# trnKhanh/medical-image-analysis

Measured on AMD Instinct MI355X. Metric: training images/sec (whole node), UNet 512x512 1ch bs=32/GPU, higher is better.
Workload: dtype bf16; 1 GPU; UNet-2D channels [64, 128, 256, 512, 1024] 512x512 1ch, batch 32/GPU, instance norm, dropout 0.1, Dice+CE, Adam(wd 5e-4), clip 10 (cfg3); global_batch=32, parallelism=dp1

## Files before the change

medical-image-analysis_amd/csrc/common.h:

```cpp
#pragma once
#include <hip/hip_runtime.h>
#include <stdint.h>
#include <stdio.h>
#include <string.h>

#define MIA_F32 0
#define MIA_BF16 1

#define MIA_OK 0
#define MIA_EARG (-1)
#define MIA_EUNSUPPORTED (-2)

extern "C" const char* mia_last_error(void);
void mia_set_error(const char* fmt, ...);

#define MIA_CHECK_ARG(cond, ...)            \
  do {                                      \
    if (!(cond)) {                          \
      mia_set_error(__VA_ARGS__);           \
      return MIA_EARG;                      \
    }                                       \
  } while (0)

#define MIA_LAUNCH_CHECK()                                                  \
// ... 134 lines not shown

__device__ __forceinline__ float wave_sum(float v) {
#pragma unroll
  for (int o = 32; o > 0; o >>= 1) v += __shfl_xor(v, o, 64);
  return v;
}

__device__ __forceinline__ double wave_sum_d(double v) {
#pragma unroll
  for (int o = 32; o > 0; o >>= 1) v += __shfl_xor(v, o, 64);
  return v;
}

__device__ __forceinline__ int wave_sum_i(int v) {
#pragma unroll
  for (int o = 32; o > 0; o >>= 1) v += __shfl_xor(v, o, 64);
  return v;
}

__device__ __forceinline__ float block_sum(float v, float* red ) {
  v = wave_sum(v);
  const int w = threadIdx.x >> 6, l = threadIdx.x & 63, nw = (blockDim.x + 63) >> 6;
  __syncthreads();
  if (l == 0) red[w] = v;
  __syncthreads();
  float r = 0.f;
  if (threadIdx.x < 64) {
    r = (l < nw) ? red[l] : 0.f;
    r = wave_sum(r);
  }
  return r;
}

static inline int ceil_div(int a, int b) { return (a + b - 1) / b; }
static inline int64_t ceil_div64(int64_t a, int64_t b) { return (a + b - 1) / b; }
```

medical-image-analysis_amd/csrc/head.hip:

```cpp
#include "common.h"

#define MAXK 8

template <typename T>
__global__ void head_fwd_kernel(const T* __restrict__ x, const float* __restrict__ w, const float* __restrict__ b,
                                float* __restrict__ out, int64_t npix, int c0, int k1, int64_t osp, int64_t osk,
                                int64_t osn, int64_t hw, bool vec) {
  extern __shared__ float wsh[];
  for (int i = threadIdx.x; i < k1 * c0; i += blockDim.x) wsh[i] = w[i];
  __syncthreads();
  constexpr int EPU = Elem<T>::EPU;
  const int sub = threadIdx.x & 7;
  for (int64_t p = ((int64_t)blockIdx.x * blockDim.x + threadIdx.x) >> 3; p < npix; p += ((int64_t)gridDim.x * blockDim.x) >> 3) {
    float acc[MAXK];
#pragma unroll
    for (int k = 0; k < MAXK; ++k) acc[k] = 0.f;
    const T* row = x + p * c0;
    if (vec) {
      for (int u = sub; u < c0 / EPU; u += 8) {
        alignas(16) T v[EPU];
        *reinterpret_cast<u32x4*>(v) = *reinterpret_cast<const u32x4*>(row + u * EPU);
#pragma unroll
        for (int e = 0; e < EPU; ++e) {
          const float xv = Elem<T>::ld(v + e);
#pragma unroll
          for (int k = 0; k < MAXK; ++k)
            if (k < k1) acc[k] += xv * wsh[k * c0 + u * EPU + e];
        }
      }
    } else {
      for (int ch = sub; ch < c0; ch += 8) {
        const float xv = Elem<T>::ld(row + ch);
#pragma unroll
// ... 164 lines not shown
  return upp;
}
#define HEAD_DISPATCH(KERNEL, T, grid, ...)                                                                           \
  do {                                                                                                                \
    if (upp == 4) {                                                                                                   \
      if (k1 == 2) hipLaunchKernelGGL((KERNEL<T, 2, 4>), grid, dim3(256), 0, st, __VA_ARGS__);                        \
      else if (k1 == 3) hipLaunchKernelGGL((KERNEL<T, 3, 4>), grid, dim3(256), 0, st, __VA_ARGS__);                   \
      else hipLaunchKernelGGL((KERNEL<T, 4, 4>), grid, dim3(256), 0, st, __VA_ARGS__);                                \
    } else if (upp == 8) {                                                                                            \
      if (k1 == 2) hipLaunchKernelGGL((KERNEL<T, 2, 8>), grid, dim3(256), 0, st, __VA_ARGS__);                        \
      else if (k1 == 3) hipLaunchKernelGGL((KERNEL<T, 3, 8>), grid, dim3(256), 0, st, __VA_ARGS__);                   \
      else hipLaunchKernelGGL((KERNEL<T, 4, 8>), grid, dim3(256), 0, st, __VA_ARGS__);                                \
    } else {                                                                                                          \
      if (k1 == 2) hipLaunchKernelGGL((KERNEL<T, 2, 16>), grid, dim3(256), 0, st, __VA_ARGS__);                       \
      else if (k1 == 3) hipLaunchKernelGGL((KERNEL<T, 3, 16>), grid, dim3(256), 0, st, __VA_ARGS__);                  \
      else hipLaunchKernelGGL((KERNEL<T, 4, 16>), grid, dim3(256), 0, st, __VA_ARGS__);                               \
    }                                                                                                                 \
  } while (0)

#define HEAD_DISPATCH_N(KERNEL, T, grid, ...)                                                                         \
  do {                                                                                                                \
    if (upp == 12) {                                                                                                  \
      if (k1 == 2) hipLaunchKernelGGL((KERNEL<T, 2, 16, 12>), grid, dim3(256), 0, st, __VA_ARGS__);                   \
      else if (k1 == 3) hipLaunchKernelGGL((KERNEL<T, 3, 16, 12>), grid, dim3(256), 0, st, __VA_ARGS__);              \
      else hipLaunchKernelGGL((KERNEL<T, 4, 16, 12>), grid, dim3(256), 0, st, __VA_ARGS__);                           \
    } else HEAD_DISPATCH(KERNEL, T, grid, __VA_ARGS__);                                                               \
  } while (0)


template <typename T, int K1, int UPP, int CU = UPP>
__global__ __launch_bounds__(256) void head_norm_fwd_kernel(const T* __restrict__ y, const float* __restrict__ scale,
                                                            const float* __restrict__ shift, float slope,
                                                            const float* __restrict__ w, const float* __restrict__ b,
                                                            float* __restrict__ out, int hw, int slabs, int64_t osn,
                                                            int64_t osp, int64_t osk) {
  constexpr int EPU = Elem<T>::EPU, C0 = CU * EPU, LANES = 256 / UPP;
  const int u = threadIdx.x % UPP, pl = threadIdx.x / UPP;
  const bool act = CU == UPP || u < CU;
  const u32x4 zero4 = {0u, 0u, 0u, 0u};
  const int n = blockIdx.x / slabs, s = blockIdx.x % slabs;
  const int per = (hw + slabs - 1) / slabs, r0 = s * per, r1 = r0 + per < hw ? r0 + per : hw;
  float wr[K1][EPU], sc[EPU], sf[EPU];
#pragma unroll
  for (int e = 0; e < EPU; ++e) {
    sc[e] = act ? scale[(size_t)n * C0 + u * EPU + e] : 0.f;
    sf[e] = act ? shift[(size_t)n * C0 + u * EPU + e] : 0.f;
#pragma unroll
    for (int k = 0; k < K1; ++k) wr[k][e] = act ? w[k * C0 + u * EPU + e] : 0.f;
  }
  float bu = 0.f;
#pragma unroll
  for (int k = 0; k < K1; ++k) bu = (u == k) ? b[k] : bu;
  const T* yb = y + (size_t)n * hw * C0 + u * EPU;
  float* ob = out + (int64_t)n * osn + u * osk;
  auto body = [&](const u32x4& raw, int p) {
    alignas(16) T v[EPU];
    *reinterpret_cast<u32x4*>(v) = raw;
    float acc[K1];
#pragma unroll
    for (int k = 0; k < K1; ++k) acc[k] = 0.f;
#pragma unroll
    for (int e = 0; e < EPU; ++e) {
      float xv = sc[e] * Elem<T>::ld(v + e) + sf[e];
      xv = xv > 0.f ? xv : xv * slope;
#pragma unroll
      for (int k = 0; k < K1; ++k) acc[k] += xv * wr[k][e];
    }
    float mine = 0.f;
#pragma unroll
    for (int k = 0; k < K1; ++k) { const float t = group_sum<UPP>(acc[k]); mine = (u == k) ? t : mine; }
    if (u < K1) ob[(int64_t)p * osp] = mine + bu;
  };
  constexpr int GP = 64 / UPP;
  __shared__ float tbuf[4][K1][64];
// ... 326 lines not shown
    if (dtype == MIA_BF16) {
      if (dx) hipLaunchKernelGGL(head_bwd_input_vec_kernel<bf16_t>, dim3(vblocks), dim3(256), k1 * c0 * 4, st, dlogits, w, static_cast<bf16_t*>(dx), npix, c0, k1, gsp, gsk, gsn, hw);
      if (wg) { hipLaunchKernelGGL(head_bwd_weight_vec_kernel<bf16_t>, dim3(wblocks), dim3(256), (256 / (c0 / epu)) * (c0 + 1) * 4, st, dlogits, static_cast<const bf16_t*>(x), workspace, npix, c0, k1, gsp, gsk, gsn, hw); }
    } else {
      if (dx) hipLaunchKernelGGL(head_bwd_input_vec_kernel<float>, dim3(vblocks), dim3(256), k1 * c0 * 4, st, dlogits, w, static_cast<float*>(dx), npix, c0, k1, gsp, gsk, gsn, hw);
      if (wg) { hipLaunchKernelGGL(head_bwd_weight_vec_kernel<float>, dim3(wblocks), dim3(256), (256 / (c0 / epu)) * (c0 + 1) * 4, st, dlogits, static_cast<const float*>(x), workspace, npix, c0, k1, gsp, gsk, gsn, hw); }
    }
  } else if (dtype == MIA_BF16) {
    if (dx) hipLaunchKernelGGL(head_bwd_input_kernel<bf16_t>, dim3(blocks), dim3(256), k1 * c0 * 4, st, dlogits, w, static_cast<bf16_t*>(dx), npix, c0, k1, gsp, gsk, gsn, hw);
    if (wg) { hipLaunchKernelGGL(head_bwd_weight_kernel<bf16_t>, dim3(wblocks), dim3(256), 512 * 4, st, dlogits, static_cast<const bf16_t*>(x), workspace, npix, c0, k1, gsp, gsk, gsn, hw); }
  } else if (dtype == MIA_F32) {
    if (dx) hipLaunchKernelGGL(head_bwd_input_kernel<float>, dim3(blocks), dim3(256), k1 * c0 * 4, st, dlogits, w, static_cast<float*>(dx), npix, c0, k1, gsp, gsk, gsn, hw);
    if (wg) { hipLaunchKernelGGL(head_bwd_weight_kernel<float>, dim3(wblocks), dim3(256), 512 * 4, st, dlogits, static_cast<const float*>(x), workspace, npix, c0, k1, gsp, gsk, gsn, hw); }
  } else { mia_set_error("mia_head_bwd: bad dtype"); return MIA_EARG; }
  if (wg) { hipLaunchKernelGGL(head_bwd_final_kernel, dim3(ceil_div(k1 * (c0 + 1), 16)), dim3(256), 0, st, workspace, wblocks, k1, c0, dw, db, accumulate); }
  MIA_LAUNCH_CHECK();
  return MIA_OK;
}

extern "C" int mia_head_norm_eligible(int dtype, int n, int64_t hw, int c0, int k1) {
  const int epu = dtype == MIA_BF16 ? 8 : 4;
  if ((dtype != MIA_BF16 && dtype != MIA_F32) || c0 % epu != 0) return 0;
  const int upp = c0 / epu;
  if ((upp != 4 && upp != 8 && upp != 12 && upp != 16) || k1 < 2 || k1 > 4) return 0;
  if (hw >= ((int64_t)1 << 31) || n > HEAD_BWD_BLOCKS) return 0;
  return upp;
}
static int head_norm_slabs(int n, int64_t hw) {
  int64_t sl = HEAD_BWD_BLOCKS / n;
  const int64_t maxsl = hw / 512 > 0 ? hw / 512 : 1;
  if (sl > maxsl) sl = maxsl;
  return (int)(sl < 1 ? 1 : sl);
}

extern "C" int mia_head_norm_fwd(const void* y, int dtype, const float* scale, const float* shift, float slope, const float* w,
                                 const float* b, float* logits, int n, int64_t hw, int c0, int k1, int64_t osn, int64_t osk,
                                 int64_t osp, void* stream) {
  MIA_CHECK_ARG(y && scale && shift && w && b && logits && n > 0 && hw > 0, "mia_head_norm_fwd: bad arguments");
  const int upp = mia_head_norm_eligible(dtype, n, hw, c0, k1);
  MIA_CHECK_ARG(upp > 0 && (reinterpret_cast<uintptr_t>(y) & 15) == 0, "mia_head_norm_fwd: shape not eligible (c0=%d k1=%d)", c0, k1);
  hipStream_t st = static_cast<hipStream_t>(stream);
  const int slabs = head_norm_slabs(n, hw);
  if (dtype == MIA_BF16) HEAD_DISPATCH_N(head_norm_fwd_kernel, bf16_t, dim3(n * slabs), static_cast<const bf16_t*>(y), scale, shift, slope, w, b, logits, (int)hw, slabs, osn, osp, osk);
  else HEAD_DISPATCH_N(head_norm_fwd_kernel, float, dim3(n * slabs), static_cast<const float*>(y), scale, shift, slope, w, b, logits, (int)hw, slabs, osn, osp, osk);
  MIA_LAUNCH_CHECK();
  return MIA_OK;
}

extern "C" int mia_head_norm_wgrad(const float* dlogits, const void* y, int dtype, const float* scale, const float* shift,
                                   float slope, float* dw, float* db, float* workspace, int n, int64_t hw, int c0, int k1,
                                   int64_t gsn, int64_t gsk, int64_t gsp, int accumulate, void* stream) {
  MIA_CHECK_ARG(dlogits && y && scale && shift && dw && db && workspace && n > 0 && hw > 0, "mia_head_norm_wgrad: bad arguments");
  const int upp = mia_head_norm_eligible(dtype, n, hw, c0, k1);
  MIA_CHECK_ARG(upp > 0 && (reinterpret_cast<uintptr_t>(y) & 15) == 0, "mia_head_norm_wgrad: shape not eligible (c0=%d k1=%d)", c0, k1);
  hipStream_t st = static_cast<hipStream_t>(stream);
  const int slabs = head_norm_slabs(n, hw);
  if (dtype == MIA_BF16) HEAD_DISPATCH_N(head_norm_wgrad_kernel, bf16_t, dim3(n * slabs), dlogits, static_cast<const bf16_t*>(y), scale, shift, slope, workspace, (int)hw, slabs, gsn, gsp, gsk);
  else HEAD_DISPATCH_N(head_norm_wgrad_kernel, float, dim3(n * slabs), dlogits, static_cast<const float*>(y), scale, shift, slope, workspace, (int)hw, slabs, gsn, gsp, gsk);
  hipLaunchKernelGGL(head_bwd_final_kernel, dim3(ceil_div(k1 * (c0 + 1), 16)), dim3(256), 0, st, workspace, n * slabs, k1, c0, dw, db, accumulate);
  MIA_LAUNCH_CHECK();
  return MIA_OK;
}
```

medical-image-analysis_amd/csrc/norm.hip:

```cpp
#include "common.h"
#include "options.h"
#include <stdlib.h>

#define NORM_INSTANCE 0
#define NORM_BATCH 1

template <bool INST>
__global__ __launch_bounds__(1024) void norm_fwd_sum_kernel(const float* __restrict__ part, int tiles, int c, float* __restrict__ xa, float* __restrict__ xb,
                                    int64_t hw, const float* __restrict__ drop, const float* __restrict__ gamma,
                                    const float* __restrict__ beta, float eps, float* __restrict__ scale, float* __restrict__ shift,
                                    float* __restrict__ ysum) {
  __shared__ double sh1[16][17], sh2[16][17];
  const int cl = threadIdx.x & 15, tl = threadIdx.x >> 4;
  const int n = blockIdx.x, ch = blockIdx.y * 16 + cl;
  double s1 = 0.0, s2 = 0.0;
  if (ch < c) {
    typedef float f2_t __attribute__((ext_vector_type(2)));
    const f2_t* p = reinterpret_cast<const f2_t*>(part) + (size_t)n * tiles * c + ch;
    int t = tl;
    for (; t + 192 < tiles; t += 256) {
      const f2_t v0 = p[(size_t)t * c], v1 = p[(size_t)(t + 64) * c], v2 = p[(size_t)(t + 128) * c], v3 = p[(size_t)(t + 192) * c];
      s1 += (double)v0.x + (double)v1.x + (double)v2.x + (double)v3.x;
      s2 += (double)v0.y + (double)v1.y + (double)v2.y + (double)v3.y;
    }
// ... 871 lines not shown
    float gv[K1];
#pragma unroll
    for (int k = 0; k < K1; ++k) gv[k] = gb[(int64_t)r * gsp + k * gsk];
    body(*reinterpret_cast<const u32x4*>(yb + (size_t)r * c), gv);
  }
#pragma unroll
  for (int e = 0; e < EPU; ++e) { sh[0][pl][u * EPU + e] = s1[e]; sh[1][pl][u * EPU + e] = s2[e]; }
  __syncthreads();
  if (threadIdx.x < 2 * CG) {
    const int k = threadIdx.x / CG, chl = threadIdx.x % CG;
    float t = 0.f;
#pragma unroll 8
    for (int j = 0; j < LANES; ++j) t += sh[k][j][chl];
    part[(((size_t)n * slabs + s) * c + blockIdx.y * CG + chl) * 2 + k] = t;
  }
  if constexpr (HWG) {
#pragma unroll
    for (int k = 0; k < K1; ++k) {
      __syncthreads();
#pragma unroll
      for (int e = 0; e < EPU; ++e) sh[0][pl][u * EPU + e] = wacc[k][e];
      if (u == 0) sh[0][pl][CG] = bacc[k];
      __syncthreads();
      if (threadIdx.x <= CG) {
        float t = 0.f;
#pragma unroll 8
        for (int j = 0; j < LANES; ++j) t += sh[0][j][threadIdx.x];
        wpart[((size_t)blockIdx.x * K1 + k) * (CG + 1) + threadIdx.x] = t;
      }
    }
  }
}

__global__ void head_w_final_kernel(const float* __restrict__ part, int nblk, int k1, int c0, float* __restrict__ dw, float* __restrict__ db,
                                    int accumulate) {
  __shared__ float sh[16][17];
  const int cl = threadIdx.x & 15, tl = threadIdx.x >> 4;
  const int i = blockIdx.x * 16 + cl, tot = k1 * (c0 + 1);
  float sm = 0.f;
  if (i < tot)
    for (int b = tl; b < nblk; b += 16) sm += part[(size_t)b * tot + i];
  sh[tl][cl] = sm;
  __syncthreads();
  if (tl == 0 && i < tot) {
    float t = 0.f;
    for (int j = 0; j < 16; ++j) t += sh[j][cl];
    const int kk = i / (c0 + 1), ch = i % (c0 + 1);
    if (ch < c0) dw[kk * c0 + ch] = accumulate ? dw[kk * c0 + ch] + t : t;
    else db[kk] = accumulate ? db[kk] + t : t;
  }
}



template <typename T, int K1>
__global__ __launch_bounds__(256) void norm_act_bwd_stream_head_kernel(const float* __restrict__ dl, const float* __restrict__ w,
                                                                       const T* __restrict__ y, T* __restrict__ dy,
                                                                       const float* __restrict__ scale, const float* __restrict__ shift,
                                                                       const float* __restrict__ xa, const float* __restrict__ xb,
                                                                       const float* __restrict__ c1, const float* __restrict__ c2,
                                                                       int hw, int c, int slabs, int upb, float slope, int64_t gsn,
                                                                       int64_t gsp, int64_t gsk, unsigned* __restrict__ amax) {
  constexpr int EPU = Elem<T>::EPU;
  const int n = blockIdx.x / slabs, s = blockIdx.x % slabs;
  const int lanes = 256 / upb;
  const int u = blockIdx.y * upb + threadIdx.x % upb, pl = threadIdx.x / upb;
  const bool live = u * EPU < c;
  if (!live && (sizeof(T) != 4 || amax == nullptr)) return;
  const int per = (hw + slabs - 1) / slabs, r0 = s * per, r1 = live ? (r0 + per < hw ? r0 + per : hw) : r0;
  float sc[EPU], sf[EPU], ka[EPU], kb[EPU], wr[K1][EPU];
  unsigned am = 0;
#pragma unroll
  for (int e = 0; e < EPU; ++e) {
    const size_t o = live ? (size_t)n * c + u * EPU + e : 0;
    sc[e] = scale[o]; sf[e] = shift[o];
    ka[e] = -sc[e] * c2[o] * xa[o];
    kb[e] = -sc[e] * (c1[o] + c2[o] * xb[o]);
#pragma unroll
    for (int k = 0; k < K1; ++k) wr[k][e] = live ? w[k * c + u * EPU + e] : 0.f;
// ... 21 lines not shown
  for (; r + 3 * lanes < r1; r += 4 * lanes) {
    u32x4 raw[4];
    float gv[4][K1];
#pragma unroll
    for (int j = 0; j < 4; ++j) raw[j] = *reinterpret_cast<const u32x4*>(y + base + (size_t)(r + j * lanes) * c);
#pragma unroll
    for (int j = 0; j < 4; ++j)
#pragma unroll
      for (int k = 0; k < K1; ++k) gv[j][k] = gb[(int64_t)(r + j * lanes) * gsp + k * gsk];
#pragma unroll
    for (int j = 0; j < 4; ++j) body(raw[j], gv[j], r + j * lanes);
  }
  for (; r < r1; r += lanes) {
    float gv[K1];
#pragma unroll
    for (int k = 0; k < K1; ++k) gv[k] = gb[(int64_t)r * gsp + k * gsk];
    body(*reinterpret_cast<const u32x4*>(y + base + (size_t)r * c), gv, r);
  }
  if constexpr (sizeof(T) == 4) { if (amax != nullptr) amax_publish(am, amax); }
}

static int norm_act_bwd_head_run(const char* who, const float* dlogits, const float* w, int k1, int64_t gsn, int64_t gsk, int64_t gsp,
                                 const NormBwd& p, float* wpart, float* dwh, float* dbh, int acc_head) {
  if (int e = bwd_check(who, p, dlogits && w && p.y && p.dy, true, true)) return e;
  MIA_CHECK_ARG(p.hw < ((int64_t)1 << 31) && k1 >= 2 && k1 <= 4 && p.c % 32 == 0, "%s: bad shape (c=%d k1=%d)", who, p.c, k1);
  MIA_CHECK_ARG(((reinterpret_cast<uintptr_t>(p.y) | reinterpret_cast<uintptr_t>(p.dy)) & 15) == 0, "%s: unaligned", who);
  const int n = p.n, c = p.c, slabs = p.slabs, dtype = p.dtype, epu = dtype == MIA_BF16 ? 8 : 4;
  const int64_t hw = p.hw; hipStream_t st = p.st;
#define CRH(T, K, CGW, HG) hipLaunchKernelGGL((colreduce_head_kernel<T, K, CGW, HG>), dim3(n * slabs, c / CGW), dim3(256), 0, st, dlogits, w, \
                                              static_cast<const T*>(p.y), p.scale, p.shift, p.xa, p.xb, (int)hw, c, slabs, p.slope, gsn, gsp, gsk, p.partials, wpart)
#define CRHK(T, CGW, HG) do { if (k1 == 2) CRH(T, 2, CGW, HG); else if (k1 == 3) CRH(T, 3, CGW, HG); else CRH(T, 4, CGW, HG); } while (0)
  if (wpart != nullptr) {
    if (dtype == MIA_BF16) CRHK(bf16_t, 64, true); else CRHK(float, 64, true);
    hipLaunchKernelGGL(head_w_final_kernel, dim3(ceil_div(k1 * (c + 1), 16)), dim3(256), 0, st, wpart, n * slabs, k1, c, dwh, dbh, acc_head);
  }
  else if (c % 64 == 0) { if (dtype == MIA_BF16) CRHK(bf16_t, 64, false); else CRHK(float, 64, false); }
  else { if (dtype == MIA_BF16) CRHK(bf16_t, 32, false); else CRHK(float, 32, false); }
#undef CRHK
#undef CRH
  bwd_finalize_launch(p);
  int sl, upb, gy;
  stream_geometry(n, hw, c, epu, &sl, &upb, &gy);
  void* amax_out = dtype == MIA_F32 ? p.amax_out : nullptr;
#define BSH(T, K) hipLaunchKernelGGL((norm_act_bwd_stream_head_kernel<T, K>), dim3(n * sl, gy), dim3(256), 0, st, dlogits, w, \
                                     static_cast<const T*>(p.y), static_cast<T*>(p.dy), p.scale, p.shift, p.xa, p.xb, p.c1, p.c2, (int)hw, c, sl, upb, \
                                     p.slope, gsn, gsp, gsk, static_cast<unsigned*>(amax_out))
#define BSHK(T) do { if (k1 == 2) BSH(T, 2); else if (k1 == 3) BSH(T, 3); else BSH(T, 4); } while (0)
  if (dtype == MIA_BF16) BSHK(bf16_t); else BSHK(float);
#undef BSHK
#undef BSH
  MIA_LAUNCH_CHECK();
  return MIA_OK;
}

extern "C" int mia_norm_act_bwd_head(const float* dlogits, const float* w, int k1, int64_t gsn, int64_t gsk, int64_t gsp,
                                     const void* y, void* dy, int dtype, const float* scale, const float* shift, const float* xa,
                                     const float* xb, const float* ysum, int n, int64_t hw, int c, int mode, int fixed_stats,
                                     float slope, int slabs, float* partials, float* c1, float* c2, float* dgamma, float* dbeta,
                                     float* dbias, int accumulate, void* amax_out, void* stream) {
  const NormBwd p{nullptr, nullptr, y, dy, dtype, scale, shift, xa, xb, ysum, n, hw, c, mode, fixed_stats, slope, slabs, partials, c1, c2,
                  dgamma, dbeta, dbias, accumulate, amax_out, static_cast<hipStream_t>(stream)};
  return norm_act_bwd_head_run("mia_norm_act_bwd_head", dlogits, w, k1, gsn, gsk, gsp, p, nullptr, nullptr, nullptr, 0);
}

extern "C" int mia_head_w_supported(int dtype, int c, int k1) {
  return ((dtype == MIA_BF16 || dtype == MIA_F32) && c == 64 && k1 >= 2 && k1 <= 4) ? 1 : 0;
}
// ... 14 lines not shown
```

medical-image-analysis_amd/csrc/stem.hip:

```cpp
#include "common.h"
#include "options.h"
#include <stdlib.h>

template <typename T, typename TI>
__global__ __launch_bounds__(256) void stem_fwd_kernel(const TI* __restrict__ x, const float* __restrict__ w ,
                                                       const float* __restrict__ bias, T* __restrict__ y, int h, int wd, int c0,
                                                       int slabs, float* __restrict__ stats ) {
  constexpr int EPU = Elem<T>::EPU;
  extern __shared__ float red[];
  const int upp = c0 / EPU, lanes = 256 / upp;
  const int u = threadIdx.x % upp, pl = threadIdx.x / upp;
  const int n = blockIdx.x / slabs, s = blockIdx.x % slabs;
  const int hw = h * wd, per = (hw + slabs - 1) / slabs, r0 = s * per, r1 = r0 + per < hw ? r0 + per : hw;
  const TI* img = x + (size_t)n * hw;
  float wr[9][EPU], br[EPU];
#pragma unroll
  for (int e = 0; e < EPU; ++e) {
    const int co = u * EPU + e;
    br[e] = bias ? bias[co] : 0.f;
#pragma unroll
    for (int t = 0; t < 9; ++t) wr[t][e] = w[co * 9 + t];
  }
  float s1[EPU], s2[EPU];
#pragma unroll
// ... 13 lines not shown
#pragma unroll
      for (int e = 0; e < EPU; ++e) {
        float a = br[e];
#pragma unroll
        for (int t = 0; t < 9; ++t) a += xv[t] * wr[t][e];
        s1[e] += a; s2[e] += a * a;
        out[e] = Elem<T>::cvt(a);
      }
      *reinterpret_cast<u32x4*>(yrow + (size_t)p * c0) = *reinterpret_cast<const u32x4*>(out);
      px += lanes;
      while (px >= wd) { px -= wd; ++py; }
    }
  }
  if (stats != nullptr) {
    if (pl < lanes)
#pragma unroll
      for (int e = 0; e < EPU; ++e) { red[pl * c0 + u * EPU + e] = s1[e]; red[(lanes + pl) * c0 + u * EPU + e] = s2[e]; }
    __syncthreads();
    for (int i = threadIdx.x; i < 2 * c0; i += 256) {
      const int k = i / c0, ch = i % c0;
      float t = 0.f;
      for (int j = 0; j < lanes; ++j) t += red[(k * lanes + j) * c0 + ch];
      stats[(((size_t)n * slabs + s) * c0 + ch) * 2 + k] = t;
    }
  }
}

typedef __amdgpu_buffer_rsrc_t srsrc_t;
template <typename T, int MT>
__global__ __launch_bounds__(256) void stem_fwd_mfma_kernel(const float* __restrict__ x, const float* __restrict__ w ,
                                                            const float* __restrict__ bias, T* __restrict__ y, int h, int wd,
                                                            int slabs, float* __restrict__ stats ) {
  constexpr int C0 = 16 * MT;
  __shared__ float red[4][2][C0];
  __shared__ __attribute__((aligned(16))) unsigned char tbuf[4 * 16 * (2 * C0 + 16)];
  const int tid = threadIdx.x, lane = tid & 63;
  const int wave = __builtin_amdgcn_readfirstlane(tid >> 6);
  const int q = lane >> 4, c16 = lane & 15;
  const int n = blockIdx.x / slabs, s = blockIdx.x % slabs;
  const int band = (h + slabs - 1) / slabs, rb = s * band, re = rb + band < h ? rb + band : h;
  const int strips = (wd + 15) / 16;
  const size_t hw = (size_t)h * wd;
  const srsrc_t rs = __builtin_amdgcn_make_buffer_rsrc(const_cast<float*>(x + (size_t)n * hw), 0, (int)(hw * 4), 0x00020000);
  float wa[MT][3];
  f32x4 bv[MT];
#pragma unroll
  for (int m = 0; m < MT; ++m) {
#pragma unroll
    for (int g = 0; g < 3; ++g) { const int t = 4 * g + q; wa[m][g] = t < 9 ? w[(16 * m + c16) * 9 + t] : 0.f; }
#pragma unroll
    for (int r = 0; r < 4; ++r) bv[m][r] = bias ? bias[16 * m + 4 * q + r] : 0.f;
  }
  int tdy[3], tdx[3];
  bool tok[3];
#pragma unroll
  for (int g = 0; g < 3; ++g) { const int t = 4 * g + q; tok[g] = t < 9; tdy[g] = (t < 9 ? t / 3 : 1) - 1; tdx[g] = (t < 9 ? t % 3 : 1) - 1; }
  float s1[MT][4], s2[MT][4];
#pragma unroll
  for (int m = 0; m < MT; ++m)
#pragma unroll
    for (int r = 0; r < 4; ++r) { s1[m][r] = 0.f; s2[m][r] = 0.f; }
  const int units = (re > rb ? re - rb : 0) * strips;
  T* yimg = y + (size_t)n * hw * C0;
  auto load_b = [&](int u, float* b) {
    const int row = rb + u / strips, x0 = (u % strips) * 16;
#pragma unroll
    for (int g = 0; g < 3; ++g) {
      const int yy = row + tdy[g], xx = x0 + c16 + tdx[g];
      const bool ok = u < units && tok[g] && (unsigned)yy < (unsigned)h && (unsigned)xx < (unsigned)wd;
      b[g] = __builtin_bit_cast(float, __builtin_amdgcn_raw_buffer_load_b32(rs, ok ? (yy * wd + xx) * 4 : (int)0xFFFFFFF0u, 0, 0));
    }
  };
  float bnext[3];
  load_b(wave, bnext);
  for (int u = wave; u < units; u += 4) {
    const int row = rb + u / strips, x0 = (u % strips) * 16;
    float b[3] = {bnext[0], bnext[1], bnext[2]};
    load_b(u + 4, bnext);
    f32x4 acc[MT];
#pragma unroll
    for (int m = 0; m < MT; ++m) {
      acc[m] = __builtin_amdgcn_mfma_f32_16x16x4f32(wa[m][0], b[0], bv[m], 0, 0, 0);
      acc[m] = __builtin_amdgcn_mfma_f32_16x16x4f32(wa[m][1], b[1], acc[m], 0, 0, 0);
      acc[m] = __builtin_amdgcn_mfma_f32_16x16x4f32(wa[m][2], b[2], acc[m], 0, 0, 0);
    }
    const bool colok = x0 + c16 < wd;
    const float msk = colok ? 1.f : 0.f;
#pragma unroll
    for (int m = 0; m < MT; ++m)
#pragma unroll
      for (int r = 0; r < 4; ++r) { const float v = acc[m][r] * msk; s1[m][r] += v; s2[m][r] += v * acc[m][r]; }
    const size_t pix = (size_t)row * wd + x0 + c16;
    if constexpr (sizeof(T) == 4) {
      if (colok)
#pragma unroll
        for (int m = 0; m < MT; ++m) *reinterpret_cast<f32x4*>(yimg + pix * C0 + 16 * m + 4 * q) = acc[m];
    } else {
      typedef __bf16 bf2_t __attribute__((ext_vector_type(2)));
      typedef float f2_t __attribute__((ext_vector_type(2)));
      typedef __attribute__((ext_vector_type(2))) unsigned int u32x2;
      auto pk = [](float a, float c) { return __builtin_bit_cast(unsigned, __builtin_convertvector(f2_t{a, c}, bf2_t)); };
      if constexpr ((MT & 1) == 0) {
        constexpr int PITCH = 2 * C0 + 16;
        unsigned char* t = tbuf + wave * (16 * PITCH);
#pragma unroll
        for (int m = 0; m < MT; ++m)
          *reinterpret_cast<u32x2*>(t + c16 * PITCH + 32 * m + 8 * q) = u32x2{pk(acc[m][0], acc[m][1]), pk(acc[m][2], acc[m][3])};
        __builtin_amdgcn_wave_barrier();
        constexpr int UPP = 2 * MT;
#pragma unroll
        for (int it = 0; it < UPP * 16 / 64; ++it) {
          const int idx = lane + 64 * it, pxl = idx / UPP, ch = idx - pxl * UPP;
          const u32x4 d = *reinterpret_cast<const u32x4*>(t + pxl * PITCH + 16 * ch);
          if (x0 + pxl < wd) *reinterpret_cast<u32x4*>(yimg + ((size_t)row * wd + x0 + pxl) * C0 + 8 * ch) = d;
        }
        __builtin_amdgcn_wave_barrier();
      } else {
#pragma unroll
        for (int m = 0; m < MT; ++m) {
          const u32x2 d = {pk(acc[m][0], acc[m][1]), pk(acc[m][2], acc[m][3])};
          if (colok) *reinterpret_cast<u32x2*>(yimg + pix * C0 + 16 * m + 4 * q) = d;
        }
      }
    }
  }
  if (stats != nullptr) {
#pragma unroll
    for (int m = 0; m < MT; ++m)
#pragma unroll
      for (int r = 0; r < 4; ++r) {
        float a = s1[m][r], c = s2[m][r];
#pragma unroll
        for (int o = 1; o < 16; o <<= 1) { a += __shfl_xor(a, o, 64); c += __shfl_xor(c, o, 64); }
        if (c16 == 0) { red[wave][0][16 * m + 4 * q + r] = a; red[wave][1][16 * m + 4 * q + r] = c; }
      }
    __syncthreads();
    for (int i = tid; i < 2 * C0; i += 256) {
      const int k = i / C0, ch = i % C0;
      stats[(((size_t)n * slabs + s) * C0 + ch) * 2 + k] = red[0][k][ch] + red[1][k][ch] + red[2][k][ch] + red[3][k][ch];
    }
  }
}

struct StemFuse {
  const void* y; const float* scale; const float* shift; const float* xa; const float* xb; const float* c1; const float* c2; float slope;
};

template <typename T, typename TI, bool FUSED = false>
__global__ __launch_bounds__(256) void stem_wgrad_kernel(const TI* __restrict__ x, const T* __restrict__ dy, float* __restrict__ part,
                                                         int slabs, int h, int wd, int c0, int win_rows, StemFuse fz) {
  constexpr int EPU = Elem<T>::EPU;
  extern __shared__ float red[];
  const int upp = c0 / EPU, lanes = 256 / upp;
  const int u = threadIdx.x % upp, pl = threadIdx.x / upp;
// ... 76 lines not shown
    int p = r0 + pl;
    int py = p / wd, px = p - py * wd;
    for (; p < r1; p += lanes) {
      float gf[EPU];
      u32x4 yraw = u32x4{0u, 0u, 0u, 0u};
      if constexpr (FUSED) yraw = *reinterpret_cast<const u32x4*>(yrow + (size_t)p * c0);
      grad_of(*reinterpret_cast<const u32x4*>(grow + (size_t)p * c0), yraw, gf);
#pragma unroll
      for (int t = 0; t < 9; ++t) {
        const int yy = py + t / 3 - 1, xx = px + t % 3 - 1;
        const float xv = ((unsigned)yy < (unsigned)h && (unsigned)xx < (unsigned)wd) ? Elem<TI>::ld(img + yy * wd + xx) : 0.f;
#pragma unroll
        for (int e = 0; e < EPU; ++e) acc[t][e] += xv * gf[e];
      }
      px += lanes;
      while (px >= wd) { px -= wd; ++py; }
    }
  }
  const int shs = c0 + 1;
  for (int t = 0; t < 9; ++t) {
    __syncthreads();
    if (pl < lanes)
#pragma unroll
      for (int e = 0; e < EPU; ++e) red[pl * shs + u * EPU + e] = acc[t][e];
    __syncthreads();
    if (threadIdx.x < c0) {
      float sm = 0.f;
      for (int j = 0; j < lanes; ++j) sm += red[j * shs + threadIdx.x];
      part[((size_t)blockIdx.x * 9 + t) * c0 + threadIdx.x] = sm;
    }
  }
}

__global__ void stem_wgrad_final_kernel(const float* __restrict__ part, int nblk, int c0, float* __restrict__ grad, int accumulate) {
  __shared__ float sh[16][17];
  const int cl = threadIdx.x & 15, tl = threadIdx.x >> 4;
  const int i = blockIdx.x * 16 + cl, tot = 9 * c0;
  float s = 0.f;
  if (i < tot)
    for (int b = tl; b < nblk; b += 16) s += part[(size_t)b * tot + i];
  sh[tl][cl] = s;
  __syncthreads();
  if (tl == 0 && i < tot) {
    float t = 0.f;
    for (int j = 0; j < 16; ++j) t += sh[j][cl];
    const int tap = i / c0, co = i % c0;
    grad[co * 9 + tap] = accumulate ? grad[co * 9 + tap] + t : t;
  }
}

#define STEM_SLABS 128
#define STEM_WBLOCKS 2048
extern "C" int mia_stem_slabs(void) { return STEM_SLABS; }
extern "C" int mia_stem_wgrad_workspace(int c0) { return STEM_WBLOCKS * 9 * c0; }

static bool stem_ok(int dtype, int c0) {
  const int epu = dtype == MIA_BF16 ? 8 : 4;
  return c0 % epu == 0 && c0 / epu <= 256 && c0 <= 256;
}

extern "C" int mia_stem_fwd(const void* x, int x_dtype, const float* w, const float* bias, void* y, int dtype, float* stat_partials,
                            int n, int h, int wd, int c0, void* stream) {
  MIA_CHECK_ARG(x && w && y && n > 0 && h > 0 && wd > 0 && c0 > 0, "mia_stem_fwd: bad arguments");
  MIA_CHECK_ARG((dtype == MIA_BF16 || dtype == MIA_F32) && (x_dtype == MIA_BF16 || x_dtype == MIA_F32), "mia_stem_fwd: bad dtype");
  MIA_CHECK_ARG(stem_ok(dtype, c0), "mia_stem_fwd: c0=%d must be a multiple of the 16-byte unit and <= 256", c0);
  const int epu = dtype == MIA_BF16 ? 8 : 4, lanes = 256 / (c0 / epu);
  MIA_CHECK_ARG((int64_t)h * wd < ((int64_t)1 << 31), "mia_stem_fwd: image too large");
  const size_t shb = (size_t)(2 * lanes * c0) * 4;
  hipStream_t st = static_cast<hipStream_t>(stream);
  dim3 grid(n * STEM_SLABS);
  const int use_mfma = mia_options().stem_mfma;
  const bool al16 = (reinterpret_cast<uintptr_t>(y) & 15) == 0;
  if (use_mfma && x_dtype == MIA_F32 && al16 && (c0 == 16 || c0 == 32 || c0 == 64 || c0 == 96 || c0 == 128) && (int64_t)h * wd * 4 < ((int64_t)1 << 31)) {
#define SM(T, MT) hipLaunchKernelGGL((stem_fwd_mfma_kernel<T, MT>), grid, dim3(256), 0, st, static_cast<const float*>(x), w, bias, static_cast<T*>(y), h, wd, STEM_SLABS, stat_partials)
#define SMT(T) do { if (c0 == 16) SM(T, 1); else if (c0 == 32) SM(T, 2); else if (c0 == 64) SM(T, 4); else if (c0 == 96) SM(T, 6); else SM(T, 8); } while (0)
    if (dtype == MIA_BF16) SMT(bf16_t); else SMT(float);
#undef SMT
#undef SM
// ... 3 lines not shown
#define SF(T, TI) hipLaunchKernelGGL((stem_fwd_kernel<T, TI>), grid, dim3(256), shb, st, static_cast<const TI*>(x), w, bias, static_cast<T*>(y), h, wd, c0, STEM_SLABS, stat_partials)
  if (dtype == MIA_BF16 && x_dtype == MIA_F32) SF(bf16_t, float);
  else if (dtype == MIA_BF16) SF(bf16_t, bf16_t);
  else if (x_dtype == MIA_F32) SF(float, float);
  else SF(float, bf16_t);
#undef SF
  MIA_LAUNCH_CHECK();
  return MIA_OK;
}

static int stem_wgrad_run(const void* x, int x_dtype, const void* dy, int dtype, float* workspace, float* grad, int n, int h, int wd,
                          int c0, int accumulate, void* stream, const StemFuse* fuse) {
  const int epu = dtype == MIA_BF16 ? 8 : 4, lanes = 256 / (c0 / epu);
  const int64_t hw = (int64_t)h * wd;
  int slabs = STEM_WBLOCKS / n;
  if (slabs > (int)((hw + 255) / 256)) slabs = (int)((hw + 255) / 256);
  if (slabs < 1) slabs = 1;
  const int blocks = n * slabs;
  hipStream_t st = static_cast<hipStream_t>(stream);
  size_t shb = (size_t)lanes * (c0 + 1) * 4;
  const int64_t per = (hw + slabs - 1) / slabs;
  int win_rows = (int)((per + wd - 1) / wd) + 3;
  if ((size_t)win_rows * (wd + 2) * 4 + shb <= 60 * 1024) shb += (size_t)win_rows * (wd + 2) * 4;
  else win_rows = 0;
  const StemFuse fz = fuse ? *fuse : StemFuse{};
#define SW(T, TI, F) hipLaunchKernelGGL((stem_wgrad_kernel<T, TI, F>), dim3(blocks), dim3(256), shb, st, static_cast<const TI*>(x), static_cast<const T*>(dy), workspace, slabs, h, wd, c0, win_rows, fz)
#define SWF(T, TI) do { if (fuse) SW(T, TI, true); else SW(T, TI, false); } while (0)
  if (dtype == MIA_BF16 && x_dtype == MIA_F32) SWF(bf16_t, float);
  else if (dtype == MIA_BF16) SWF(bf16_t, bf16_t);
  else if (x_dtype == MIA_F32) SWF(float, float);
  else SWF(float, bf16_t);
#undef SWF
#undef SW
  hipLaunchKernelGGL(stem_wgrad_final_kernel, dim3(ceil_div(9 * c0, 16)), dim3(256), 0, st, workspace, blocks, c0, grad, accumulate);
  MIA_LAUNCH_CHECK();
  return MIA_OK;
}

extern "C" int mia_stem_wgrad(const void* x, int x_dtype, const void* dy, int dtype, float* workspace, float* grad, int n, int h, int wd,
                              int c0, int accumulate, void* stream) {
  MIA_CHECK_ARG(x && dy && workspace && grad && n > 0 && h > 0 && wd > 0, "mia_stem_wgrad: bad arguments");
  MIA_CHECK_ARG((dtype == MIA_BF16 || dtype == MIA_F32) && (x_dtype == MIA_BF16 || x_dtype == MIA_F32), "mia_stem_wgrad: bad dtype");
  MIA_CHECK_ARG(stem_ok(dtype, c0), "mia_stem_wgrad: c0=%d must be a multiple of the 16-byte unit and <= 256", c0);
  MIA_CHECK_ARG((int64_t)h * wd < ((int64_t)1 << 31) && n <= STEM_WBLOCKS, "mia_stem_wgrad: image or batch too large");
  return stem_wgrad_run(x, x_dtype, dy, dtype, workspace, grad, n, h, wd, c0, accumulate, stream, nullptr);
}

extern "C" int mia_stem_wgrad_fused(const void* x, int x_dtype, const void* dz, const void* y, int dtype, const float* scale,
                                    const float* shift, const float* xa, const float* xb, const float* c1, const float* c2, float slope,
                                    float* workspace, float* grad, int n, int h, int wd, int c0, int accumulate, void* stream) {
  MIA_CHECK_ARG(x && dz && y && scale && shift && xa && xb && c1 && c2 && workspace && grad && n > 0 && h > 0 && wd > 0,
                "mia_stem_wgrad_fused: bad arguments");
  MIA_CHECK_ARG((dtype == MIA_BF16 || dtype == MIA_F32) && (x_dtype == MIA_BF16 || x_dtype == MIA_F32), "mia_stem_wgrad_fused: bad dtype");
  MIA_CHECK_ARG(stem_ok(dtype, c0), "mia_stem_wgrad_fused: c0=%d must be a multiple of the 16-byte unit and <= 256", c0);
  MIA_CHECK_ARG((int64_t)h * wd < ((int64_t)1 << 31) && n <= STEM_WBLOCKS, "mia_stem_wgrad_fused: image or batch too large");
  MIA_CHECK_ARG(((reinterpret_cast<uintptr_t>(dz) | reinterpret_cast<uintptr_t>(y)) & 15) == 0, "mia_stem_wgrad_fused: dz / y must be 16-byte aligned");
  const StemFuse fz{y, scale, shift, xa, xb, c1, c2, slope};
  return stem_wgrad_run(x, x_dtype, dz, dtype, workspace, grad, n, h, wd, c0, accumulate, stream, &fz);
}
```

Baseline: 784.1 images/sec.

## Widen final column reductions, unroll stem forward, and align head-forward slabs

```diff
diff --git a/medical-image-analysis_amd/csrc/common.h b/medical-image-analysis_amd/csrc/common.h
--- a/medical-image-analysis_amd/csrc/common.h
+++ b/medical-image-analysis_amd/csrc/common.h
@@ -190,5 +190,37 @@
   return r;
 }
 
+#define FINAL_COLS 16
+#define FINAL_LANES 64
+#define FINAL_THREADS (FINAL_COLS * FINAL_LANES)
+__device__ __forceinline__ float final_column_sum(const float* __restrict__ part, int nblk, int tot, int i) {
+  __shared__ float sh[FINAL_LANES][FINAL_COLS + 1];
+  __shared__ float sh4[4][FINAL_COLS + 1];
+  const int cl = threadIdx.x % FINAL_COLS, tl = threadIdx.x / FINAL_COLS;
+  float s = 0.f;
+  if (i < tot) {
+    const float* col = part + i;
+    int b = tl;
+    for (; b + 7 * FINAL_LANES < nblk; b += 8 * FINAL_LANES) {
+      float v[8];
+#pragma unroll
+      for (int j = 0; j < 8; ++j) v[j] = col[(size_t)(b + j * FINAL_LANES) * tot];
+#pragma unroll
+      for (int j = 0; j < 8; ++j) s += v[j];
+    }
+    for (; b < nblk; b += FINAL_LANES) s += col[(size_t)b * tot];
+  }
+  sh[tl][cl] = s;
+  __syncthreads();
+  if (tl < 4) {
+    float t = 0.f;
+#pragma unroll
+    for (int j = 0; j < 16; ++j) t += sh[tl * 16 + j][cl];
+    sh4[tl][cl] = t;
+  }
+  __syncthreads();
+  return tl == 0 ? ((sh4[0][cl] + sh4[1][cl]) + sh4[2][cl]) + sh4[3][cl] : 0.f;
+}
+
 static inline int ceil_div(int a, int b) { return (a + b - 1) / b; }
 static inline int64_t ceil_div64(int64_t a, int64_t b) { return (a + b - 1) / b; }
diff --git a/medical-image-analysis_amd/csrc/head.hip b/medical-image-analysis_amd/csrc/head.hip
--- a/medical-image-analysis_amd/csrc/head.hip
+++ b/medical-image-analysis_amd/csrc/head.hip
@@ -1,4 +1,5 @@
 #include "common.h"
+#include "options.h"
 
 #define MAXK 8
 
@@ -229,14 +230,14 @@
 __global__ __launch_bounds__(256) void head_norm_fwd_kernel(const T* __restrict__ y, const float* __restrict__ scale,
                                                             const float* __restrict__ shift, float slope,
                                                             const float* __restrict__ w, const float* __restrict__ b,
-                                                            float* __restrict__ out, int hw, int slabs, int64_t osn,
+                                                            float* __restrict__ out, int hw, int slabs, int per, int64_t osn,
                                                             int64_t osp, int64_t osk) {
   constexpr int EPU = Elem<T>::EPU, C0 = CU * EPU, LANES = 256 / UPP;
   const int u = threadIdx.x % UPP, pl = threadIdx.x / UPP;
   const bool act = CU == UPP || u < CU;
   const u32x4 zero4 = {0u, 0u, 0u, 0u};
   const int n = blockIdx.x / slabs, s = blockIdx.x % slabs;
-  const int per = (hw + slabs - 1) / slabs, r0 = s * per, r1 = r0 + per < hw ? r0 + per : hw;
+  const int r0 = s * per, r1 = r0 + per < hw ? r0 + per : hw;
   float wr[K1][EPU], sc[EPU], sf[EPU];
 #pragma unroll
   for (int e = 0; e < EPU; ++e) {
@@ -629,6 +630,16 @@
   if (sl > maxsl) sl = maxsl;
   return (int)(sl < 1 ? 1 : sl);
 }
+static void head_fwd_slabs(int n, int64_t hw, int* slabs, int* per) {
+  int64_t sl = mia_options().stream_blocks / n;
+  const int64_t maxsl = hw / 512 > 0 ? hw / 512 : 1;
+  if (sl > maxsl) sl = maxsl;
+  if (sl < 1) sl = 1;
+  int64_t p = (hw + sl - 1) / sl;
+  if (sl > 1) p = (p + 255) / 256 * 256;
+  *per = (int)p;
+  *slabs = (int)((hw + p - 1) / p);
+}
 
 extern "C" int mia_head_norm_fwd(const void* y, int dtype, const float* scale, const float* shift, float slope, const float* w,
                                  const float* b, float* logits, int n, int64_t hw, int c0, int k1, int64_t osn, int64_t osk,
@@ -637,9 +648,10 @@
   const int upp = mia_head_norm_eligible(dtype, n, hw, c0, k1);
   MIA_CHECK_ARG(upp > 0 && (reinterpret_cast<uintptr_t>(y) & 15) == 0, "mia_head_norm_fwd: shape not eligible (c0=%d k1=%d)", c0, k1);
   hipStream_t st = static_cast<hipStream_t>(stream);
-  const int slabs = head_norm_slabs(n, hw);
-  if (dtype == MIA_BF16) HEAD_DISPATCH_N(head_norm_fwd_kernel, bf16_t, dim3(n * slabs), static_cast<const bf16_t*>(y), scale, shift, slope, w, b, logits, (int)hw, slabs, osn, osp, osk);
-  else HEAD_DISPATCH_N(head_norm_fwd_kernel, float, dim3(n * slabs), static_cast<const float*>(y), scale, shift, slope, w, b, logits, (int)hw, slabs, osn, osp, osk);
+  int slabs, per;
+  head_fwd_slabs(n, hw, &slabs, &per);
+  if (dtype == MIA_BF16) HEAD_DISPATCH_N(head_norm_fwd_kernel, bf16_t, dim3(n * slabs), static_cast<const bf16_t*>(y), scale, shift, slope, w, b, logits, (int)hw, slabs, per, osn, osp, osk);
+  else HEAD_DISPATCH_N(head_norm_fwd_kernel, float, dim3(n * slabs), static_cast<const float*>(y), scale, shift, slope, w, b, logits, (int)hw, slabs, per, osn, osp, osk);
   MIA_LAUNCH_CHECK();
   return MIA_OK;
 }
diff --git a/medical-image-analysis_amd/csrc/norm.hip b/medical-image-analysis_amd/csrc/norm.hip
--- a/medical-image-analysis_amd/csrc/norm.hip
+++ b/medical-image-analysis_amd/csrc/norm.hip
@@ -927,19 +927,11 @@
   }
 }
 
-__global__ void head_w_final_kernel(const float* __restrict__ part, int nblk, int k1, int c0, float* __restrict__ dw, float* __restrict__ db,
-                                    int accumulate) {
-  __shared__ float sh[16][17];
-  const int cl = threadIdx.x & 15, tl = threadIdx.x >> 4;
-  const int i = blockIdx.x * 16 + cl, tot = k1 * (c0 + 1);
-  float sm = 0.f;
-  if (i < tot)
-    for (int b = tl; b < nblk; b += 16) sm += part[(size_t)b * tot + i];
-  sh[tl][cl] = sm;
-  __syncthreads();
-  if (tl == 0 && i < tot) {
-    float t = 0.f;
-    for (int j = 0; j < 16; ++j) t += sh[j][cl];
+__global__ __launch_bounds__(FINAL_THREADS) void head_w_final_kernel(const float* __restrict__ part, int nblk, int k1, int c0,
+                                                                     float* __restrict__ dw, float* __restrict__ db, int accumulate) {
+  const int i = blockIdx.x * FINAL_COLS + threadIdx.x % FINAL_COLS, tot = k1 * (c0 + 1);
+  const float t = final_column_sum(part, nblk, tot, i);
+  if (threadIdx.x < FINAL_COLS && i < tot) {
     const int kk = i / (c0 + 1), ch = i % (c0 + 1);
     if (ch < c0) dw[kk * c0 + ch] = accumulate ? dw[kk * c0 + ch] + t : t;
     else db[kk] = accumulate ? db[kk] + t : t;
@@ -1027,7 +1019,7 @@
 #define CRHK(T, CGW, HG) do { if (k1 == 2) CRH(T, 2, CGW, HG); else if (k1 == 3) CRH(T, 3, CGW, HG); else CRH(T, 4, CGW, HG); } while (0)
   if (wpart != nullptr) {
     if (dtype == MIA_BF16) CRHK(bf16_t, 64, true); else CRHK(float, 64, true);
-    hipLaunchKernelGGL(head_w_final_kernel, dim3(ceil_div(k1 * (c + 1), 16)), dim3(256), 0, st, wpart, n * slabs, k1, c, dwh, dbh, acc_head);
+    hipLaunchKernelGGL(head_w_final_kernel, dim3(ceil_div(k1 * (c + 1), FINAL_COLS)), dim3(FINAL_THREADS), 0, st, wpart, n * slabs, k1, c, dwh, dbh, acc_head);
   }
   else if (c % 64 == 0) { if (dtype == MIA_BF16) CRHK(bf16_t, 64, false); else CRHK(float, 64, false); }
   else { if (dtype == MIA_BF16) CRHK(bf16_t, 32, false); else CRHK(float, 32, false); }
diff --git a/medical-image-analysis_amd/csrc/stem.hip b/medical-image-analysis_amd/csrc/stem.hip
--- a/medical-image-analysis_amd/csrc/stem.hip
+++ b/medical-image-analysis_amd/csrc/stem.hip
@@ -69,8 +69,11 @@
                                                             const float* __restrict__ bias, T* __restrict__ y, int h, int wd,
                                                             int slabs, float* __restrict__ stats ) {
   constexpr int C0 = 16 * MT;
+  constexpr int UN = MT <= 4 ? 2 : 1;
+  constexpr int PITCH = 2 * C0 + 16;
+  constexpr bool TRANSPOSE = sizeof(T) == 2 && (MT & 1) == 0;
   __shared__ float red[4][2][C0];
-  __shared__ __attribute__((aligned(16))) unsigned char tbuf[4 * 16 * (2 * C0 + 16)];
+  __shared__ __attribute__((aligned(16))) unsigned char tbuf[TRANSPOSE ? 4 * 2 * UN * 16 * PITCH : 16];
   const int tid = threadIdx.x, lane = tid & 63;
   const int wave = __builtin_amdgcn_readfirstlane(tid >> 6);
   const int q = lane >> 4, c16 = lane & 15;
@@ -108,55 +111,87 @@
       b[g] = __builtin_bit_cast(float, __builtin_amdgcn_raw_buffer_load_b32(rs, ok ? (yy * wd + xx) * 4 : (int)0xFFFFFFF0u, 0, 0));
     }
   };
-  float bnext[3];
-  load_b(wave, bnext);
-  for (int u = wave; u < units; u += 4) {
-    const int row = rb + u / strips, x0 = (u % strips) * 16;
-    float b[3] = {bnext[0], bnext[1], bnext[2]};
-    load_b(u + 4, bnext);
-    f32x4 acc[MT];
-#pragma unroll
-    for (int m = 0; m < MT; ++m) {
-      acc[m] = __builtin_amdgcn_mfma_f32_16x16x4f32(wa[m][0], b[0], bv[m], 0, 0, 0);
-      acc[m] = __builtin_amdgcn_mfma_f32_16x16x4f32(wa[m][1], b[1], acc[m], 0, 0, 0);
-      acc[m] = __builtin_amdgcn_mfma_f32_16x16x4f32(wa[m][2], b[2], acc[m], 0, 0, 0);
-    }
-    const bool colok = x0 + c16 < wd;
-    const float msk = colok ? 1.f : 0.f;
+  float bn[UN][3];
+#pragma unroll
+  for (int k = 0; k < UN; ++k) load_b(wave + 4 * k, bn[k]);
+  int par = 0;
+  for (int u = wave; u < units; u += 4 * UN) {
+    float b[UN][3];
+#pragma unroll
+    for (int k = 0; k < UN; ++k)
+#pragma unroll
+      for (int g = 0; g < 3; ++g) b[k][g] = bn[k][g];
+#pragma unroll
+    for (int k = 0; k < UN; ++k) load_b(u + 4 * (UN + k), bn[k]);
+    f32x4 acc[UN][MT];
 #pragma unroll
     for (int m = 0; m < MT; ++m)
 #pragma unroll
-      for (int r = 0; r < 4; ++r) { const float v = acc[m][r] * msk; s1[m][r] += v; s2[m][r] += v * acc[m][r]; }
-    const size_t pix = (size_t)row * wd + x0 + c16;
+      for (int k = 0; k < UN; ++k) acc[k][m] = __builtin_amdgcn_mfma_f32_16x16x4f32(wa[m][0], b[k][0], bv[m], 0, 0, 0);
+#pragma unroll
+    for (int g = 1; g < 3; ++g)
+#pragma unroll
+      for (int m = 0; m < MT; ++m)
+#pragma unroll
+        for (int k = 0; k < UN; ++k) acc[k][m] = __builtin_amdgcn_mfma_f32_16x16x4f32(wa[m][g], b[k][g], acc[k][m], 0, 0, 0);
+    int row[UN], x0[UN];
+    bool live[UN], colok[UN];
+#pragma unroll
+    for (int k = 0; k < UN; ++k) {
+      const int uk = u + 4 * k;
+      row[k] = rb + uk / strips; x0[k] = (uk % strips) * 16;
+      live[k] = uk < units; colok[k] = live[k] && x0[k] + c16 < wd;
+      const float msk = colok[k] ? 1.f : 0.f;
+#pragma unroll
+      for (int m = 0; m < MT; ++m)
+#pragma unroll
+        for (int r = 0; r < 4; ++r) {
+          const float v = acc[k][m][r] * msk;
+          s1[m][r] += v; s2[m][r] = __builtin_fmaf(v, acc[k][m][r], s2[m][r]);
+        }
+    }
     if constexpr (sizeof(T) == 4) {
-      if (colok)
-#pragma unroll
-        for (int m = 0; m < MT; ++m) *reinterpret_cast<f32x4*>(yimg + pix * C0 + 16 * m + 4 * q) = acc[m];
+#pragma unroll
+      for (int k = 0; k < UN; ++k) {
+        const size_t pix = (size_t)row[k] * wd + x0[k] + c16;
+        if (colok[k])
+#pragma unroll
+          for (int m = 0; m < MT; ++m) *reinterpret_cast<f32x4*>(yimg + pix * C0 + 16 * m + 4 * q) = acc[k][m];
+      }
     } else {
       typedef __bf16 bf2_t __attribute__((ext_vector_type(2)));
       typedef float f2_t __attribute__((ext_vector_type(2)));
       typedef __attribute__((ext_vector_type(2))) unsigned int u32x2;
       auto pk = [](float a, float c) { return __builtin_bit_cast(unsigned, __builtin_convertvector(f2_t{a, c}, bf2_t)); };
       if constexpr ((MT & 1) == 0) {
-        constexpr int PITCH = 2 * C0 + 16;
-        unsigned char* t = tbuf + wave * (16 * PITCH);
-#pragma unroll
-        for (int m = 0; m < MT; ++m)
-          *reinterpret_cast<u32x2*>(t + c16 * PITCH + 32 * m + 8 * q) = u32x2{pk(acc[m][0], acc[m][1]), pk(acc[m][2], acc[m][3])};
+        unsigned char* t = tbuf + ((wave * 2 + par) * UN) * (16 * PITCH);
+        par ^= 1;
+#pragma unroll
+        for (int k = 0; k < UN; ++k)
+#pragma unroll
+          for (int m = 0; m < MT; ++m)
+            *reinterpret_cast<u32x2*>(t + k * (16 * PITCH) + c16 * PITCH + 32 * m + 8 * q) = u32x2{pk(acc[k][m][0], acc[k][m][1]), pk(acc[k][m][2], acc[k][m][3])};
         __builtin_amdgcn_wave_barrier();
         constexpr int UPP = 2 * MT;
 #pragma unroll
-        for (int it = 0; it < UPP * 16 / 64; ++it) {
-          const int idx = lane + 64 * it, pxl = idx / UPP, ch = idx - pxl * UPP;
-          const u32x4 d = *reinterpret_cast<const u32x4*>(t + pxl * PITCH + 16 * ch);
-          if (x0 + pxl < wd) *reinterpret_cast<u32x4*>(yimg + ((size_t)row * wd + x0 + pxl) * C0 + 8 * ch) = d;
-        }
-        __builtin_amdgcn_wave_barrier();
+        for (int k = 0; k < UN; ++k)
+#pragma unroll
+          for (int it = 0; it < UPP * 16 / 64; ++it) {
+            const int idx = lane + 64 * it, pxl = idx / UPP, ch = idx - pxl * UPP;
+            const u32x4 d = *reinterpret_cast<const u32x4*>(t + k * (16 * PITCH) + pxl * PITCH + 16 * ch);
+            store_data_fence();
+            if (live[k] && x0[k] + pxl < wd) *reinterpret_cast<u32x4*>(yimg + ((size_t)row[k] * wd + x0[k] + pxl) * C0 + 8 * ch) = d;
+            store_data_pad();
+          }
       } else {
 #pragma unroll
-        for (int m = 0; m < MT; ++m) {
-          const u32x2 d = {pk(acc[m][0], acc[m][1]), pk(acc[m][2], acc[m][3])};
-          if (colok) *reinterpret_cast<u32x2*>(yimg + pix * C0 + 16 * m + 4 * q) = d;
+        for (int k = 0; k < UN; ++k) {
+          const size_t pix = (size_t)row[k] * wd + x0[k] + c16;
+#pragma unroll
+          for (int m = 0; m < MT; ++m) {
+            const u32x2 d = {pk(acc[k][m][0], acc[k][m][1]), pk(acc[k][m][2], acc[k][m][3])};
+            if (colok[k]) *reinterpret_cast<u32x2*>(yimg + pix * C0 + 16 * m + 4 * q) = d;
+          }
         }
       }
     }
@@ -299,18 +334,11 @@
   }
 }
 
-__global__ void stem_wgrad_final_kernel(const float* __restrict__ part, int nblk, int c0, float* __restrict__ grad, int accumulate) {
-  __shared__ float sh[16][17];
-  const int cl = threadIdx.x & 15, tl = threadIdx.x >> 4;
-  const int i = blockIdx.x * 16 + cl, tot = 9 * c0;
-  float s = 0.f;
-  if (i < tot)
-    for (int b = tl; b < nblk; b += 16) s += part[(size_t)b * tot + i];
-  sh[tl][cl] = s;
-  __syncthreads();
-  if (tl == 0 && i < tot) {
-    float t = 0.f;
-    for (int j = 0; j < 16; ++j) t += sh[j][cl];
+__global__ __launch_bounds__(FINAL_THREADS) void stem_wgrad_final_kernel(const float* __restrict__ part, int nblk, int c0,
+                                                                         float* __restrict__ grad, int accumulate) {
+  const int i = blockIdx.x * FINAL_COLS + threadIdx.x % FINAL_COLS, tot = 9 * c0;
+  const float t = final_column_sum(part, nblk, tot, i);
+  if (threadIdx.x < FINAL_COLS && i < tot) {
     const int tap = i / c0, co = i % c0;
     grad[co * 9 + tap] = accumulate ? grad[co * 9 + tap] + t : t;
   }
@@ -380,7 +408,7 @@
   else SWF(float, bf16_t);
 #undef SWF
 #undef SW
-  hipLaunchKernelGGL(stem_wgrad_final_kernel, dim3(ceil_div(9 * c0, 16)), dim3(256), 0, st, workspace, blocks, c0, grad, accumulate);
+  hipLaunchKernelGGL(stem_wgrad_final_kernel, dim3(ceil_div(9 * c0, FINAL_COLS)), dim3(FINAL_THREADS), 0, st, workspace, blocks, c0, grad, accumulate);
   MIA_LAUNCH_CHECK();
   return MIA_OK;
 }
```

Measured after the change: 782.6 images/sec. Within noise of the previous version (-0.2%).
